# Chainscore/dot-ring

Measured on AMD Instinct MI355X. Metric: ringvrf_proofs_per_sec, higher is better.
Workload: dtype u32

## Files before the change

dot_ring_amd/csrc/capi_msm.hip:

```cpp
#include "capi_internal.hpp"
#include "kernels_g1.hip.h"
#include "kernels_te_msm.hip.h"

using namespace dri;

static MsmKnobs msm_knobs() {
    static const int force_groups = std::getenv("DOTRING_MSM_GROUPS") ? std::atoi(std::getenv("DOTRING_MSM_GROUPS")) : 0;
    static const bool naf_tiling = !(std::getenv("DOTRING_SRS_TILING") && std::strcmp(std::getenv("DOTRING_SRS_TILING"), "rows") == 0);
    return MsmKnobs{g_force_c, force_groups, naf_tiling};
}

namespace {
int msm_reserve(dr_ctx* ctx, const MsmPlan& p) {
    const auto& b = p.bytes;
    for (const auto& r : {std::make_pair(&ctx->counts, b.counts), {&ctx->offsets, b.offsets}, {&ctx->tiles, b.tiles}, {&ctx->perm, b.perm},
                          {&ctx->cells, b.cells}, {&ctx->cell_off, b.cell_off}, {&ctx->buckets, b.buckets}, {&ctx->partial, b.partial},
                          {&ctx->winsum, b.winsum}, {&ctx->heavy, b.heavy}, {&ctx->sorted, b.sorted}, {&ctx->digits, b.digits},
                          {&ctx->cursor, b.cursor}, {&ctx->part_base, b.part_base}, {&ctx->result, b.result}})
        TRY(r.first->reserve(r.second));
    return DR_OK;
}

void exclusive_scan(dr_ctx* ctx, const uint32_t* in, uint32_t* out, size_t count) {
    hipStream_t st = ctx->stream;
    const unsigned nt = div_up(count, dr::SCAN_TILE);
    hipLaunchKernelGGL(dr::k_scan_tiles, dim3(nt), dim3(dr::SCAN_BLOCK), 0, st, in, out, ctx->tiles.as<uint32_t>(), count);
    hipLaunchKernelGGL(dr::k_scan_tile_sums, dim3(1), dim3(dr::SCAN_BLOCK), 0, st, ctx->tiles.as<uint32_t>(), nt, ctx->tiles.as<uint32_t>() + nt);
    hipLaunchKernelGGL(dr::k_scan_add, dim3(div_up(count, 256)), dim3(256), 0, st, out, ctx->tiles.as<uint32_t>(), count);
}

int msm_sort(dr_ctx* ctx, const MsmPlan& p, const uint32_t* d_scalars, const MsmTable* tbl, bool exact, const uint32_t*& part_flag) {
    hipStream_t st = ctx->stream;
    if (p.sort == MsmSort::sets || p.sort == MsmSort::sets_staged) {
        dr::SortSetParams sp{};
        sp.n = (uint32_t)p.n; sp.batch = (uint32_t)p.batch; sp.H = p.H; sp.groups = p.groups; sp.single = p.single ? 1 : 0;
        sp.tbl_stride = p.single ? tbl->stride : 0; sp.tbl_offset = p.single ? tbl->offset : 0; sp.capacity = (uint32_t)p.per_set_digits;
        sp.short_from = p.single ? tbl->short_from : 0xffffffffu; sp.n_short = p.single ? std::min<uint32_t>(tbl->n_short, (uint32_t)p.n) : 0;
        sp.sets = (uint32_t)p.bsets; sp.fold = p.single && tbl->fold_sign ? 1 : 0; sp.n_pad = p.n_pad; sp.digits_per_set = p.digits_per_set;
        return launch(ctx, "k_g1_sort_sets", [&] {
            const auto staged = p.H <= dr::SORT2_SMALL_H ? dr::k_g1_sort_sets_staged<dr::SORT2_SMALL_H, dr::SORT2_CAP_SMALL_H>
                                                         : dr::k_g1_sort_sets_staged<dr::SORT_MAX_H, dr::SORT2_CAP_LARGE_H>;
            if (p.sort == MsmSort::sets_staged)
                hipLaunchKernelGGL(staged, dim3((unsigned)p.bsets), dim3(dr::SORT2_BLOCK), 0, st, d_scalars, p.wt, sp, ctx->digits.as<uint16_t>(),
                                   ctx->counts.as<uint32_t>(), ctx->offsets.as<uint32_t>(), ctx->sorted.as<uint32_t>());
            else
                hipLaunchKernelGGL(dr::k_g1_sort_sets, dim3((unsigned)p.bsets), dim3(dr::SORT_BLOCK), 0, st, d_scalars, p.wt, sp,
                                   ctx->counts.as<uint32_t>(), ctx->offsets.as<uint32_t>(), ctx->sorted.as<uint32_t>());
        });
    }
    if (p.sort == MsmSort::partition) {
        dr::PartParams pp{};
        pp.n = (uint32_t)p.n; pp.H = p.H; pp.groups = p.groups; pp.P = p.part_p; pp.pshift = p.part_shift; pp.tile = p.part_tile;
        pp.tiles_per_set = p.part_tiles_per_set; pp.cap_part = p.part_cap; pp.capacity = (uint32_t)p.per_set_digits;
        pp.tbl_stride = tbl->stride; pp.tbl_offset = tbl->offset;
        for (int w = 0; w < p.wt.W; w++) pp.row[w] = p.wt.row[w];
        const size_t nparts = p.nparts();
        uint32_t* d_flag = ctx->cursor.as<uint32_t>() + nparts;
        const uint32_t* d_exact = nullptr;
        bool fits = true;
        if (exact) {
            std::vector<uint32_t> fill(nparts), at(nparts);
            HIP_TRY(hipMemcpyAsync(fill.data(), ctx->cursor.p, nparts * 4, hipMemcpyDeviceToHost, st));
            HIP_TRY(hipStreamSynchronize(st));
            uint64_t run = 0, most = 0;
            for (size_t q = 0; q < nparts; q++) { at[q] = (uint32_t)run; run += fill[q]; most = std::max<uint64_t>(most, fill[q]); }
            fits = most <= dr::PART_MAX_CHUNKS * (dr::PART_STAGE - dr::PART_SLACK) && run <= nparts * (uint64_t)pp.cap_part;
            if (fits) {
                HIP_TRY(hipMemcpyAsync(ctx->part_base.p, at.data(), nparts * 4, hipMemcpyHostToDevice, st));
                HIP_TRY(hipStreamSynchronize(st));
                d_exact = ctx->part_base.as<uint32_t>();
            }
        }
        if (fits) {
            HIP_TRY(hipMemsetAsync(ctx->cursor.p, 0, (nparts + 1) * 4, st));
            TRY(launch(ctx, "k_g1_part_scatter", [&] {
                hipLaunchKernelGGL(dr::k_g1_part_scatter, dim3((unsigned)(p.bsets * pp.tiles_per_set)), dim3(dr::PART_BLOCK), 0, st, d_scalars, p.wt, pp,
                                   ctx->cursor.as<uint32_t>(), d_exact, ctx->digits.as<uint2>());
            }));
            if (!exact) part_flag = d_flag;
            return launch(ctx, "k_g1_part_sort", [&] {
                hipLaunchKernelGGL(dr::k_g1_part_sort, dim3((unsigned)nparts), dim3(dr::PART_BLOCK), 0, st, ctx->digits.as<uint2>(),
                                   ctx->cursor.as<uint32_t>(), d_exact, pp, d_flag, ctx->counts.as<uint32_t>(), ctx->offsets.as<uint32_t>(),
                                   ctx->sorted.as<uint32_t>());
            });
        }
    }
    HIP_TRY(hipMemsetAsync(ctx->counts.p, 0, p.nbuckets * 4, st));
    HIP_TRY(hipMemsetAsync(ctx->cursor.p, 0, p.nbuckets * 4, st));
    TRY(launch(ctx, "k_g1_digits", [&] {
        hipLaunchKernelGGL(dr::k_g1_digits, dim3(div_up(p.n * p.batch, 256)), dim3(256), 0, st, d_scalars, (uint32_t)p.n,
                           (uint32_t)p.batch, p.wt, p.single ? 1 : 0, p.groups, ctx->digits.as<int32_t>(), ctx->counts.as<uint32_t>());
    }));
    TRY(launch(ctx, "k_scan", [&] { exclusive_scan(ctx, ctx->counts.as<uint32_t>(), ctx->offsets.as<uint32_t>(), p.nbuckets); }));
    return launch(ctx, "k_g1_scatter", [&] {
        hipLaunchKernelGGL(dr::k_g1_scatter, dim3(div_up(p.ndigits, 256)), dim3(256), 0, st, ctx->digits.as<int32_t>(),
                           (uint32_t)p.n, p.windows, p.H, p.single ? p.wt.W : 0, p.wt, p.single ? tbl->stride : 0u, p.single ? tbl->offset : 0u,
// ... 891 lines not shown
```

dot_ring_amd/csrc/kernels_g1.hip.h:

```cpp
#pragma once
#include "dev_types.hpp"
#include "g1.hip.h"
#include "msm_plan.hpp"
#include "msm_recode.hip.h"

namespace dr {

__global__ __launch_bounds__(256) void k_g1_bases_to_mont(uint32_t* bases, uint32_t n) {
    uint32_t i = blockIdx.x * blockDim.x + threadIdx.x;
    if (i >= n) return;
    uint32_t* p = bases + (size_t)i * 24;
    uint32_t wx[12], wy[12];
    load_words12(p, wx);
    load_words12(p + 12, wy);
    store_fq28(p, to_mont28(wx));
    store_fq28(p + 12, to_mont28(wy));
}

__global__ __launch_bounds__(256) void k_g1_synth_bases(uint32_t* bases, uint32_t n, uint32_t first, const uint32_t* seed) {
    uint32_t i = blockIdx.x * blockDim.x + threadIdx.x;
    if (i >= n) return;
    G1Affine s = load_affine(seed, 0);
    uint32_t k = first + i;
    G1Xyzz acc = g1_inf();
// ... 313 lines not shown
    uint32_t i = (uint32_t)(gid % n);
    uint32_t mag = d < 0 ? (uint32_t)(-d) : (uint32_t)d;
    size_t bset = win;
    uint32_t entry = i;
    if (W > 0) {
        bset = (win / W) * groups + (size_t)(((uint64_t)i * groups) / n);
        entry = (uint32_t)wt.row[win % W] * tbl_stride + tbl_offset + i;
    }
    size_t bucket = bset * H + (mag - 1);
    uint32_t pos = offsets[bucket] + atomicAdd(&cursor[bucket], 1u);
    sorted[pos] = entry | (d < 0 ? 0x80000000u : 0u);
}

__global__ __launch_bounds__(256) void k_g1_window_table(const uint32_t* __restrict__ bases, uint32_t n, WindowTable wt, uint32_t pt_words, uint32_t* __restrict__ table) {
    uint32_t i = blockIdx.x * blockDim.x + threadIdx.x;
    if (i >= n) return;
    G1Affine a = load_affine(bases, i);
    G1Xyzz cur = g1_from_affine(a);
#pragma unroll 1
    for (int w = 0; w < wt.W; w++) {
        if (w > 0) {
#pragma unroll 1
            for (int j = 0; j < wt.width[w - 1]; j++) cur = g1_dbl(cur);
            a = g1_to_affine_dev(cur);
        }
        store_affine(table + ((size_t)w * n + i) * (pt_words - 24), (size_t)w * n + i, a);
    }
}

__global__ __launch_bounds__(128) void k_g1_bit_table(const uint32_t* __restrict__ bases, uint32_t n, uint32_t rows, uint32_t pt_words, uint32_t* __restrict__ table) {
    uint32_t i = blockIdx.x * blockDim.x + threadIdx.x;
    if (i >= n) return;
    G1Affine a = load_affine(bases, i);
#pragma unroll 1
    for (uint32_t s = 0; s < rows; s++) {
        if (s > 0 && !a.inf) a = g1_to_affine_dev(g1_dbl_affine(a));
        store_affine(table + ((size_t)s * n + i) * (pt_words - 24), (size_t)s * n + i, a);
    }
}

DR_DEV uint32_t digit_bin(const WindowTable& wt, int w, uint32_t mag, uint32_t& row) {
    row = wt.row[w];
    return mag - 1u;
}

constexpr int SORT_BLOCK = 256;

struct SortSetParams {
    uint32_t n, batch, H, groups;
    int single;
    uint32_t tbl_stride, tbl_offset;
    uint32_t capacity;
    uint32_t short_from, n_short;
    uint32_t n_pad, digits_per_set;
    uint32_t sets;
    int fold;
};

DR_DEV void load_scalar_mod_r(const uint32_t* __restrict__ scalars, size_t idx, uint32_t (&k)[9]) {
    const uint4* q = reinterpret_cast<const uint4*>(scalars + idx * 8);
    uint4 lo = q[0], hi = q[1];
    k[0] = lo.x; k[1] = lo.y; k[2] = lo.z; k[3] = lo.w; k[4] = hi.x; k[5] = hi.y; k[6] = hi.z; k[7] = hi.w;
    k[8] = 0;
    constexpr uint32_t R[8] = {0x00000001u, 0xffffffffu, 0xfffe5bfeu, 0x53bda402u, 0x09a1d805u, 0x3339d808u, 0x299d7d48u, 0x73eda753u};
#pragma unroll 1
    for (int it = 0; it < 2; it++) {
        uint32_t d[8], borrow = 0;
#pragma unroll
        for (int j = 0; j < 8; j++) d[j] = subb(k[j], R[j], borrow);
#pragma unroll
        for (int j = 0; j < 8; j++) k[j] = borrow ? k[j] : d[j];
    }
}

DR_DEV bool scalar_fold_sign(uint32_t (&k)[9]) {
    constexpr uint32_t R[8] = {0x00000001u, 0xffffffffu, 0xfffe5bfeu, 0x53bda402u, 0x09a1d805u, 0x3339d808u, 0x299d7d48u, 0x73eda753u};
    constexpr uint32_t HALF[8] = {0x80000000u, 0x7fffffffu, 0x7fff2dffu, 0xa9ded201u, 0x04d0ec02u, 0x199cec04u, 0x94cebea4u, 0x39f6d3a9u};
    uint32_t borrow = 0, d[8];
#pragma unroll
    for (int j = 0; j < 8; j++) (void)subb(HALF[j], k[j], borrow);
    const bool neg = borrow != 0;
    borrow = 0;
#pragma unroll
    for (int j = 0; j < 8; j++) d[j] = subb(R[j], k[j], borrow);
#pragma unroll
    for (int j = 0; j < 8; j++) k[j] = neg ? d[j] : k[j];
    return neg;
}


__global__ __launch_bounds__(SORT_BLOCK) void k_g1_sort_sets(const uint32_t* __restrict__ scalars, WindowTable wt, SortSetParams sp,
                                                             uint32_t* __restrict__ counts, uint32_t* __restrict__ offsets,
                                                             uint32_t* __restrict__ sorted) {
    __shared__ uint32_t bins[SORT_MAX_H];
    __shared__ uint32_t smem[SORT_BLOCK / 64];
    const uint32_t H = sp.H, HB = sp.H, set = blockIdx.x;
    uint32_t b, i_lo, i_hi;
    int w_lo, w_hi;
    if (sp.single) {
        b = set / sp.groups;
        uint32_t g = set % sp.groups;
        const uint32_t n_eff = b >= sp.short_from ? sp.n_short : sp.n;
        i_lo = (uint32_t)(((uint64_t)g * n_eff + sp.groups - 1) / sp.groups);
        i_hi = (uint32_t)(((uint64_t)(g + 1) * n_eff + sp.groups - 1) / sp.groups);
        w_lo = 0; w_hi = wt.W;
    } else {
        const uint32_t sw = set / sp.groups, g = set % sp.groups;
        b = sw / wt.W;
// ... 7 lines not shown
        uint32_t k[9];
        load_scalar_mod_r(scalars, (size_t)b * sp.n + i, k);
        if (sp.fold) (void)scalar_fold_sign(k);
        if (wt.odd == 2) {
            for_each_wnaf_digit(k, wt, [&](int, uint32_t, int32_t d) { atomicAdd(&bins[((uint32_t)(d < 0 ? -d : d) - 1u) >> 1], 1u); });
            continue;
        }
        for_each_digit(k, wt, w_lo, w_hi, [&](int w, int32_t d) {
            uint32_t row;
            atomicAdd(&bins[digit_bin(wt, w, (uint32_t)(d < 0 ? -d : d), row)], 1u);
        });
    }
    __syncthreads();
    const uint32_t per = (HB + SORT_BLOCK - 1) / SORT_BLOCK, lo = threadIdx.x * per < HB ? threadIdx.x * per : HB, hi = lo + per < HB ? lo + per : HB;
    uint32_t local = 0;
    for (uint32_t j = lo; j < hi; j++) {
        uint32_t c = bins[j];
        counts[(size_t)set * H + j] = c;
        local += c;
    }
    uint32_t total;
    uint32_t run = block_exclusive_scan(local, smem, total);
    const uint32_t base = set * sp.capacity;
    for (uint32_t j = lo; j < hi; j++) {
        uint32_t c = bins[j];
        bins[j] = run;
        offsets[(size_t)set * H + j] = base + run;
        run += c;
    }
    __syncthreads();
    for (uint32_t i = i_lo + threadIdx.x; i < i_hi; i += SORT_BLOCK) {
        uint32_t k[9];
        load_scalar_mod_r(scalars, (size_t)b * sp.n + i, k);
        const bool neg = sp.fold ? scalar_fold_sign(k) : false;
        if (wt.odd == 2) {
            for_each_wnaf_digit(k, wt, [&](int j, uint32_t o, int32_t d) {
                const uint32_t pos = atomicAdd(&bins[((uint32_t)(d < 0 ? -d : d) - 1u) >> 1], 1u);
                const uint32_t entry = ((uint32_t)wt.row[j] + o) * sp.tbl_stride + sp.tbl_offset + i;
                sorted[base + pos] = entry | ((d < 0) != neg ? 0x80000000u : 0u);
            });
            continue;
        }
        for_each_digit(k, wt, w_lo, w_hi, [&](int w, int32_t d) {
            uint32_t row;
            uint32_t pos = atomicAdd(&bins[digit_bin(wt, w, (uint32_t)(d < 0 ? -d : d), row)], 1u);
            uint32_t entry = sp.single ? row * sp.tbl_stride + sp.tbl_offset + i : i;
            sorted[base + pos] = entry | ((d < 0) != neg ? 0x80000000u : 0u);
        });
    }
}

template <uint32_t MAX_H, uint32_t SORT2_CAP>
__global__ __launch_bounds__(SORT2_BLOCK) void k_g1_sort_sets_staged(const uint32_t* __restrict__ scalars, WindowTable wt, SortSetParams sp,
                                                                    uint16_t* __restrict__ digits16, uint32_t* __restrict__ counts,
                                                                    uint32_t* __restrict__ offsets, uint32_t* __restrict__ sorted) {
    constexpr uint32_t SORT2_CHUNK = SORT2_CAP - SORT2_SLACK;
    __shared__ uint32_t bins[MAX_H];
    __shared__ uint32_t stage[SORT2_CAP];
    __shared__ uint32_t cs[SORT2_MAX_CHUNKS + 1], jb[SORT2_MAX_CHUNKS + 1];
    __shared__ uint32_t smem[SORT2_BLOCK / 64];
    const uint32_t H = sp.H, set = blockIdx.x, tid = threadIdx.x;
    uint32_t b, i_lo, i_hi;
    int w_lo, w_hi;
    if (sp.single) {
        b = set / sp.groups;
        uint32_t g = set % sp.groups;
        const uint32_t n_eff = b >= sp.short_from ? sp.n_short : sp.n;
        i_lo = (uint32_t)(((uint64_t)g * n_eff + sp.groups - 1) / sp.groups);
        i_hi = (uint32_t)(((uint64_t)(g + 1) * n_eff + sp.groups - 1) / sp.groups);
        w_lo = 0; w_hi = wt.W;
    } else {
        const uint32_t sw = set / sp.groups, g = set % sp.groups;
        b = sw / wt.W;
        w_lo = (int)(sw % wt.W); w_hi = w_lo + 1;
        i_lo = (uint32_t)(((uint64_t)g * sp.n + sp.groups - 1) / sp.groups);
        i_hi = (uint32_t)(((uint64_t)(g + 1) * sp.n + sp.groups - 1) / sp.groups);
    }
    const uint32_t n_set = i_hi - i_lo, n_pad = (n_set + 7u) & ~7u, rows = (uint32_t)(w_hi - w_lo);
    uint16_t* dg = digits16 + (size_t)set * sp.digits_per_set;
    for (uint32_t j = tid; j < H; j += SORT2_BLOCK) bins[j] = 0;
    for (uint32_t k = tid; k <= SORT2_MAX_CHUNKS; k += SORT2_BLOCK) { cs[k] = 0xffffffffu; jb[k] = H; }
    __syncthreads();
    for (uint32_t ii = tid; ii < n_pad; ii += SORT2_BLOCK) {
        if (ii < n_set) {
            uint32_t k[9];
            load_scalar_mod_r(scalars, (size_t)b * sp.n + i_lo + ii, k);
            const bool neg = sp.fold ? scalar_fold_sign(k) : false;
            if (wt.odd == 2) {
                for_each_wnaf_digit<true>(k, wt, [&](int j, uint32_t o, int32_t d) {
                    uint32_t enc = WNAF_EMPTY16;
                    if (d != 0) {
                        const uint32_t bin = ((uint32_t)(d < 0 ? -d : d) - 1u) >> 1;
                        atomicAdd(&bins[bin], 1u);
                        enc = bin | (o << 11) | ((d < 0) != neg ? 0x8000u : 0u);
                    }
                    dg[(size_t)j * n_pad + ii] = (uint16_t)enc;
                });
            } else
            for_each_digit<true>(k, wt, w_lo, w_hi, [&](int w, int32_t d) {
                const uint32_t mag = (uint32_t)(d < 0 ? -d : d);
                uint32_t row, enc = mag;
                if (d != 0) {
                    atomicAdd(&bins[digit_bin(wt, w, mag, row)], 1u);
                }
                dg[(size_t)(w - w_lo) * n_pad + ii] = (uint16_t)(enc | ((d < 0) != neg && d != 0 ? 0x8000u : 0u));
            });
        } else {
            for (uint32_t r = 0; r < rows; r++) dg[(size_t)r * n_pad + ii] = wt.odd == 2 ? (uint16_t)WNAF_EMPTY16 : (uint16_t)0;
        }
    }
    __syncthreads();
    const uint32_t per = (H + SORT2_BLOCK - 1) / SORT2_BLOCK, lo = tid * per < H ? tid * per : H, hi = lo + per < H ? lo + per : H;
    uint32_t local = 0;
    for (uint32_t j = lo; j < hi; j++) {
        uint32_t c = bins[j];
        counts[(size_t)set * H + j] = c;
        local += c;
    }
    uint32_t total;
    uint32_t run = block_exclusive_scan<SORT2_BLOCK>(local, smem, total);
    const uint32_t base = set * sp.capacity;
    const uint32_t K = (total + SORT2_CHUNK - 1) / SORT2_CHUNK;
    for (uint32_t j = lo; j < hi; j++) {
        uint32_t c = bins[j];
        bins[j] = run;
        offsets[(size_t)set * H + j] = base + run;
        const uint32_t k = run / SORT2_CHUNK;
        atomicMin(&jb[k], j);
        atomicMin(&cs[k], run);
        run += c;
    }
    __syncthreads();
    if (tid == 0) {
        cs[K] = total; jb[K] = H;
        for (int k = (int)K - 1; k >= 0; k--) {
            if (cs[k] == 0xffffffffu) cs[k] = cs[k + 1];
            if (jb[k] > jb[k + 1]) jb[k] = jb[k + 1];
        }
    }
    __syncthreads();
    const uint32_t tbl = sp.single ? sp.tbl_offset : 0u;
    for (uint32_t k = 0; k < K; k++) {
        const uint32_t j_lo = jb[k], j_hi = jb[k + 1], p_lo = cs[k], p_hi = cs[k + 1], c0 = k * SORT2_CHUNK;
        if (j_lo < j_hi) {
            const uint32_t nv = n_pad / 8, nvec = rows * nv;
            const uint4* vecs = reinterpret_cast<const uint4*>(dg);
            uint32_t r = 0, v = tid;
            for (uint32_t idx = tid; idx < nvec; idx += SORT2_BLOCK, v += SORT2_BLOCK) {
                while (v >= nv) { v -= nv; r++; }
                const uint32_t row_entry = (sp.single ? (uint32_t)wt.row[w_lo + (int)r] * sp.tbl_stride : 0u) + tbl + i_lo;
                {
                    const uint4 q = vecs[idx];
                    const uint32_t words[4] = {q.x, q.y, q.z, q.w};
#pragma unroll
                    for (int t = 0; t < 8; t++) {
                        const uint32_t dd = (words[t >> 1] >> (16 * (t & 1))) & 0xffffu;
                        const uint32_t j = wt.odd == 2 ? (((dd >> 11) & 15u) == 15u ? 0xffffffffu : (dd & 0x7ffu)) : (dd & 0x7fffu) - 1u;
                        if (j >= j_lo && j < j_hi) {
                            uint32_t up = 0;
                            if (wt.odd == 2) {
                                up = ((dd >> 11) & 15u) * sp.tbl_stride;
                            }
                            const uint32_t pos = atomicAdd(&bins[j], 1u);
                            const uint32_t entry = (row_entry + up + v * 8 + (uint32_t)t) | ((dd & 0x8000u) << 16);
                            const uint32_t rel = pos - c0;
                            if (rel < SORT2_CAP) stage[rel] = entry;
                            else sorted[base + pos] = entry;
                        }
                    }
                }
            }
        }
        __syncthreads();
        const uint32_t r_lo = p_lo - c0, r_hi = (p_hi - c0) < SORT2_CAP ? (p_hi - c0) : SORT2_CAP;
        for (uint32_t rel = r_lo + tid; rel < r_hi; rel += SORT2_BLOCK) sorted[base + c0 + rel] = stage[rel];
        __syncthreads();
    }
}

struct PartParams {
    uint32_t n, H, groups, tiles_per_set, P, pshift;
    uint32_t tile;
    uint32_t cap_part;
    uint32_t capacity;
    uint32_t tbl_stride, tbl_offset;
    uint8_t row[32];
};

DR_DEV void part_set_range(const PartParams& pp, uint32_t set, uint32_t& b, uint32_t& i_lo, uint32_t& i_hi) {
    b = set / pp.groups;
    const uint32_t g = set % pp.groups;
    i_lo = (uint32_t)(((uint64_t)g * pp.n + pp.groups - 1) / pp.groups);
    i_hi = (uint32_t)(((uint64_t)(g + 1) * pp.n + pp.groups - 1) / pp.groups);
}

DR_DEV uint32_t lds_count_aggregated(uint32_t* bins, uint32_t j) {
    const uint32_t lane = threadIdx.x & 63u;
    unsigned long long todo = __ballot(1);
    uint32_t pos = 0;
    bool done = false;
#pragma unroll 1
    for (int round = 0; round < 4 && todo; round++) {
        const int leader = __builtin_ctzll(todo);
        const uint32_t j0 = (uint32_t)__shfl((int)j, leader, 64);
        const unsigned long long same = __ballot(!done && j == j0);
        if (__popcll(same) < 2 && round == 0) break;
        uint32_t base = 0;
        if ((int)lane == leader) base = atomicAdd(&bins[j0], (uint32_t)__popcll(same));
        base = (uint32_t)__shfl((int)base, leader, 64);
        if (!done && j == j0) { pos = base + (uint32_t)__popcll(same & ((1ull << lane) - 1ull)); done = true; }
        todo &= ~same;
    }
    if (!done) pos = atomicAdd(&bins[j], 1u);
    return pos;
}

__global__ __launch_bounds__(PART_BLOCK) void k_g1_part_scatter(const uint32_t* __restrict__ scalars, WindowTable wt, PartParams pp,
                                                                uint32_t* __restrict__ part_fill, const uint32_t* __restrict__ exact_base,
                                                                uint2* __restrict__ streams) {
    constexpr int WAVES = PART_BLOCK / 64;
    __shared__ uint32_t stage[PART_TILE_ENTRIES];
    __shared__ uint32_t cnt[PART_MAX_P];
    __shared__ uint32_t pbase[PART_MAX_P + 1], gbase[PART_MAX_P];
    __shared__ uint32_t smem[PART_BLOCK / 64];
    const uint32_t set = blockIdx.x / pp.tiles_per_set, tile = blockIdx.x % pp.tiles_per_set, tid = threadIdx.x, wave = tid >> 6;
    const bool per_wave = pp.P * WAVES <= PART_MAX_P;
    uint32_t b, i_lo, i_hi;
    part_set_range(pp, set, b, i_lo, i_hi);
// ... 622 lines not shown
```

dot_ring_amd/csrc/msm_plan.hpp:

```cpp
#pragma once
#include <algorithm>
#include <cmath>
#include <cstddef>
#include <cstdint>

#include "dev_types.hpp"

namespace dr {

constexpr int SCAN_BLOCK = 256, SCAN_ITEMS = 8, SCAN_TILE = SCAN_BLOCK * SCAN_ITEMS;
constexpr uint32_t SORT_MAX_H = 8192;
constexpr int SORT2_BLOCK = 1024;
constexpr uint32_t SORT2_SLACK = 2048, SORT2_MAX_CHUNKS = 64;
constexpr uint32_t SORT2_CAP_SMALL_H = 36864, SORT2_CAP_LARGE_H = 28672, SORT2_SMALL_H = 2048;
constexpr int PART_BLOCK = 1024;
constexpr uint32_t PART_TILE_ENTRIES = 32768, PART_MAX_P = 1024, PART_MAX_HP = 1024, PART_STAGE = 36864, PART_SLACK = 2048, PART_MAX_CHUNKS = 64;
constexpr int SZ_BLOCK = 256, SZ_ITEMS = 8, SZ_TILE = SZ_BLOCK * SZ_ITEMS, SZ_CLASSES = 256;
constexpr uint32_t G1_HEAVY_SLOTS = 2048;
constexpr int RS_BLOCK = 64, RS_GROUP = 4;
constexpr int WS_BLOCK = 256;

constexpr int MIN_WINDOW = 7, MAX_WINDOW = 16, MAX_TABLE_WINDOW = 22;
inline bool forced_window_ok(int c) { return c >= MIN_WINDOW && c <= MAX_WINDOW; }
inline bool table_window_ok(int c) { return c >= MIN_WINDOW && c <= MAX_TABLE_WINDOW; }

inline int pick_window(size_t n) {
    int best = MIN_WINDOW;
    double best_cost = 1e300;
    for (int c = MIN_WINDOW; c <= MAX_WINDOW; c++) {
        int W = (256 + c - 1) / c;
        double cost = (double)W * ((double)n + 2.8 * (double)(1u << (c - 1)) + 40.0 * (double)((1u << (c - 1)) / 16 + 1));
        if (cost < best_cost) { best_cost = cost; best = c; }
    }
    return best;
}

inline int pick_window_latency(size_t n) {
    int best = 7;
    double best_t = 1e300;
    for (int c = 7; c <= 13; c++) {
        const int W = (256 + c - 1) / c;
        const double H = (double)(1u << (c - 1));
        if ((double)W * H > 131072.0) continue;
        const double m = (double)n / H;
        const double reduce = H >= 256.0 ? 15.0 * (2.0 * std::min(8.0, std::max(1.0, H / 1024.0)) + 17.0)
                                         : 15.0 * (8.0 + 1.5 * (c - 3)) + 15.0 * (std::log2(std::max(H / 4.0, 2.0)) + 4.0);
        const double t = 11.0 * (m + 3.0 * std::sqrt(m) + 1.0) + reduce;
        if (t < best_t) { best_t = t; best = c; }
    }
    return best;
}

inline WindowTable make_window_table(int c, int bits = 256) {
    WindowTable wt;
    wt.W = (bits + c - 1) / c;
    int base = bits / wt.W, rem = bits % wt.W;
    wt.cmax = base + (rem ? 1 : 0);
    int bit = 0;
    for (int w = 0; w < wt.W; w++) {
        int width = base + (w >= wt.W - rem ? 1 : 0);
        wt.start[w] = (uint8_t)bit, wt.width[w] = (uint8_t)width, wt.row[w] = (uint8_t)w;
        bit += width;
    }
    wt.odd = 0;
    return wt;
}

// ... 1 lines not shown

struct MsmTable {
    const uint32_t* table = nullptr;
    dr::WindowTable wt{};
    uint32_t pt_words = 24;
    bool bit_rows = false;
    int naf_delta = -2;
    uint32_t stride = 0, offset = 0;
    uint32_t short_from = 0xffffffffu, n_short = 0;
    bool fold_sign = false;
};

struct MsmKnobs { int force_c = 0, force_groups = 0; bool naf_tiling = true; };

constexpr size_t L4_BELOW = (size_t)1 << 15;

struct Tiling { bool naf; int c, slots; double digits; };

inline Tiling tiling_for(const MsmTable& t, size_t n, size_t batch, bool naf_tiling) {
    Tiling none{false, 0, 0, 0.0};
    if (!t.table || !t.bit_rows || t.naf_delta == -1 || batch < 256 || n == 0 || !naf_tiling) return none;
    const int cn = t.wt.cmax;
    const int lo = t.naf_delta >= 0 ? cn + t.naf_delta : cn - 1, hi = t.naf_delta >= 0 ? cn + t.naf_delta : cn + 2;
    Tiling best = none;
    double best_cost = 0;
    for (int w = lo; w <= hi; w++) {
        if (w < 9 || w > 13) continue;
        const size_t H = (size_t)1 << (w - 2), slots = (256 + w - 1) / w;
        if (batch * (H / 16) < L4_BELOW) continue;
        if ((n + 64) * slots > ((size_t)1 << 20) || batch * (n + 64) * slots >= (1ull << 32)) continue;
        const double digits = 256.0 / (w + 1) + 0.55;
        if (t.naf_delta < 0 && (double)n * digits / (double)H > 160.0) continue;
        const double cost = (double)n * digits + 1.5 * (double)H;
        if (!best.naf || cost < best_cost) { best = Tiling{true, w, (int)slots, digits}; best_cost = cost; }
    }
    return best;
}

enum class MsmSort { sets, sets_staged, partition, global };
enum class MsmReduce { set_scan, levels, wg_scan, chunks, chunks_two_stage };
enum class MsmFinish { group_sum, device_copy, host_horner, device_horner };

struct MsmPlan {
    const char* error = nullptr;
    size_t n = 0, batch = 0;
    bool single = false;
    dr::WindowTable wt{};
    uint32_t H = 0, L = 0, T = 0, groups = 1;
    size_t windows = 0, bsets = 0, nbuckets = 0, ndigits = 0, per_set_scalars = 0, per_set_digits = 0;
    MsmSort sort = MsmSort::global;
    MsmReduce reduce = MsmReduce::chunks;
    MsmFinish finish = MsmFinish::group_sum;
    uint32_t n_pad = 0, digits_per_set = 0;
    uint32_t part_p = 1, part_shift = 0;
    uint32_t part_tile = 0, part_tiles_per_set = 0, part_cap = 0;
    uint32_t ws_per_lane = 1, ws_span = 0;
    size_t wg_per_set = 0, wg_count = 0;
    size_t szblocks = 0, ncells = 0;
    struct { size_t counts, offsets, tiles, perm, cells, cell_off, buckets, partial, winsum, heavy, sorted, digits, cursor, part_base, result; }
        bytes{};
    size_t nparts() const { return bsets * (size_t)part_p; }
};

inline MsmPlan msm_shape(size_t n, size_t batch, const MsmTable* tbl, const MsmKnobs& k, bool allow_naf) {
    MsmPlan p;
    p.n = n, p.batch = batch, p.single = tbl != nullptr && tbl->table != nullptr;
    if (p.single) {
        const Tiling tl = allow_naf ? tiling_for(*tbl, n, batch, k.naf_tiling) : Tiling{false, 0, 0, 0.0};
        if (tl.naf) {
            const int shift = tl.slots * tl.c - 256;
            p.wt.W = tl.slots, p.wt.cmax = tl.c, p.wt.odd = 2;
            for (int j = 0; j < p.wt.W; j++)
                p.wt.start[j] = (uint8_t)(tl.c * j), p.wt.row[j] = (uint8_t)(j ? tl.c * j - shift : 0), p.wt.width[j] = (uint8_t)tl.c;
        } else {
            p.wt = tbl->wt;
        }
        p.H = 1u << (p.wt.cmax - (tl.naf ? 2 : 1));
    } else {
        const bool latency_bound = batch == 1 && n <= 32768;
        p.wt = dr::make_window_table(dr::forced_window_ok(k.force_c) ? k.force_c : latency_bound ? dr::pick_window_latency(n) : dr::pick_window(n));
        p.H = 1u << (p.wt.cmax - 1);
    }
    p.L = std::min<uint32_t>(p.H, 16u);
    if (p.single) {
        const size_t target_lanes = n >= ((size_t)1 << 19) ? 524288 : 262144;
        while (p.groups < 64 && batch * p.groups * (size_t)p.H < target_lanes && n / (p.groups * 2) >= 64) p.groups *= 2;
        if (k.force_groups > 0 && batch == 1 && n / (size_t)k.force_groups >= 64) p.groups = (uint32_t)k.force_groups;
    }
    p.windows = batch * (size_t)p.wt.W;
    p.bsets = p.single ? batch * p.groups : p.windows;
    if (p.single && p.L == 16 && p.H >= 256 && p.H <= 4096 && p.bsets * (size_t)(p.H / 16) < L4_BELOW) p.L = 4;
    if (!p.single && p.L == 16 && p.H >= 16 && p.bsets * (size_t)(p.H / 16) < ((size_t)1 << 12)) p.L = 4;
    p.T = p.H / p.L;
    p.per_set_scalars = p.single ? (n + p.groups - 1) / p.groups : n;
    p.per_set_digits = p.single ? p.per_set_scalars * (size_t)p.wt.W : n;
    const bool lds_sort = p.H <= dr::SORT_MAX_H && p.bsets >= 64 && p.per_set_digits <= (1u << 20) && p.bsets * p.per_set_digits < (1ull << 32);
    p.sort = lds_sort ? MsmSort::sets : MsmSort::global;
    const bool setscan = p.L == 16 && p.T >= 8 && p.T <= 256 && p.bsets >= 256;
    p.reduce = setscan ? MsmReduce::set_scan : MsmReduce::chunks;
    return p;
}

inline MsmPlan plan_msm(size_t n, size_t batch, const MsmTable* tbl, const MsmKnobs& k) {
    MsmPlan p = msm_shape(n, batch, tbl, k, true);
    if (p.wt.odd && !(p.sort == MsmSort::sets && p.reduce == MsmReduce::set_scan)) p = msm_shape(n, batch, tbl, k, false);
    const uint32_t H = p.H, T = p.T, W = (uint32_t)p.wt.W;
    const size_t bsets = p.bsets;
    if (p.single && ((uint64_t)p.wt.row[W - 1] + p.wt.cmax + 1) * tbl->stride >= (1ull << 31)) { p.error = "window table too large"; return p; }
    p.nbuckets = bsets * (size_t)H, p.ndigits = p.windows * n;
    if (p.nbuckets >= (1ull << 32) || p.ndigits >= (1ull << 32)) { p.error = "MSM batch too large for one launch (split the batch)"; return p; }

    if (p.sort == MsmSort::sets) {
        const uint32_t stage_chunk = (H <= dr::SORT2_SMALL_H ? dr::SORT2_CAP_SMALL_H : dr::SORT2_CAP_LARGE_H) - dr::SORT2_SLACK;
        if (p.per_set_digits >= 4096 && p.per_set_digits / stage_chunk + 1 <= dr::SORT2_MAX_CHUNKS) {
            p.sort = MsmSort::sets_staged;
            p.n_pad = (uint32_t)((p.per_set_scalars + 7) & ~(size_t)7), p.digits_per_set = p.n_pad * (p.single ? W : 1u);
        }
    }
    const size_t chunk = dr::PART_STAGE - dr::PART_SLACK;
    while (p.part_p < dr::PART_MAX_P && (H / p.part_p > dr::PART_MAX_HP || p.per_set_digits / p.part_p > chunk - chunk / 16)) p.part_p *= 2;
    while ((H >> p.part_shift) > p.part_p) p.part_shift++;
    if (p.sort == MsmSort::global && p.single && batch == 1 && W <= 32 && H >= p.part_p && H / p.part_p <= dr::PART_MAX_HP &&
        p.per_set_digits / p.part_p <= 48 * chunk && bsets * p.per_set_digits < (1ull << 32) && p.per_set_digits >= 65536) {
        p.sort = MsmSort::partition;
        p.part_tile = std::min<uint32_t>(2048, dr::PART_TILE_ENTRIES / W);
        p.part_tiles_per_set = (uint32_t)((p.per_set_scalars + p.part_tile - 1) / p.part_tile);
        p.part_cap = (uint32_t)std::min<size_t>(p.per_set_digits, std::max<size_t>(4 * p.per_set_digits / p.part_p, 65536));
    }

    const bool setscan = p.reduce == MsmReduce::set_scan;
    const bool leveled = p.L == 16 && H >= 256 && bsets * (size_t)(H / 16) >= ((size_t)1 << 18);
    const bool plain_one = !p.single && batch == 1 && !setscan && !leveled && H >= 256 && !p.wt.odd;
    if (plain_one) p.ws_per_lane = std::min<uint32_t>(8u, std::max<uint32_t>(1u, H / 1024u));
    else while (p.ws_per_lane < 8 && bsets * (size_t)H > (size_t)65536 * p.ws_per_lane) p.ws_per_lane *= 2;
    p.ws_span = dr::WS_BLOCK * p.ws_per_lane;
    const bool few_table = p.single && batch <= 32 && !setscan && !leveled && H >= 256 && !p.wt.odd && bsets * (size_t)H <= ((size_t)1 << 19);
    const bool wgscan = (plain_one || few_table || (!setscan && !leveled && p.single && batch == 1 && H >= 8192)) && H % p.ws_span == 0;
    p.wg_per_set = H / p.ws_span, p.wg_count = bsets * p.wg_per_set;
    if (!setscan) p.reduce = leveled ? MsmReduce::levels : wgscan ? MsmReduce::wg_scan
                           : T > 512 && T % 256 == 0 ? MsmReduce::chunks_two_stage : MsmReduce::chunks;
    if (p.single) p.finish = wgscan || p.groups > 1 || batch == 1 ? MsmFinish::group_sum : MsmFinish::device_copy;
    else p.finish = batch == 1 ? MsmFinish::host_horner : MsmFinish::device_horner;

    p.szblocks = (p.nbuckets + dr::SZ_TILE - 1) / dr::SZ_TILE, p.ncells = (size_t)dr::SZ_CLASSES * p.szblocks;
    auto& b = p.bytes;
    b.counts = b.perm = p.nbuckets * 4, b.offsets = (p.nbuckets + 1) * 4;
    b.tiles = (size_t)((std::max(p.ncells, p.nbuckets) + dr::SCAN_TILE - 1) / dr::SCAN_TILE + 1) * 4;
    b.cells = p.ncells * 4, b.cell_off = (p.ncells + 2) * 4;
    b.buckets = p.nbuckets * 192;
    size_t levels = 0;
    for (uint32_t m = H; m > 16; m /= 16) levels += 2 * bsets * (m / 16);
    b.partial = std::max((bsets * T + bsets * (T / 256 + 1)) * 192, p.reduce == MsmReduce::set_scan ? 2 * bsets * T * 192
                         : p.reduce == MsmReduce::wg_scan ? 2 * p.wg_count * 192 : p.reduce == MsmReduce::levels ? levels * 192 : 0);
    b.winsum = bsets * 192;
    b.heavy = (p.ndigits / 1024 + p.ndigits / 4096 + dr::G1_HEAVY_SLOTS / 2 + 64) * 192;
    const bool global = p.sort == MsmSort::global, part = p.sort == MsmSort::partition;
    b.sorted = global ? p.ndigits * 4 : bsets * p.per_set_digits * 4;
    b.digits = global ? p.ndigits * 4 : part ? p.nparts() * p.part_cap * 8 : bsets * (size_t)p.digits_per_set * 2;
    b.cursor = global ? p.nbuckets * 4 : part ? std::max(p.nparts() + 1, p.nbuckets) * 4 : 0;
    b.part_base = part ? p.nparts() * 4 : 0;
    b.result = batch > 1 ? batch * 192 : 0;
    return p;
}
```

dot_ring_amd/csrc/msm_recode.hip.h:

```cpp
#pragma once
#include <cstdint>

#include "dev_types.hpp"

#if defined(__HIPCC__)
#define DR_RECODE_FN __device__ __forceinline__
#else
#define DR_RECODE_FN static inline
#endif

namespace dr {

template <bool WITH_ZEROS = false, class F>
DR_RECODE_FN void for_each_digit(const uint32_t (&k)[9], const WindowTable& wt, int w_lo, int w_hi, F&& f) {
    uint32_t carry = 0;
    int w = 0;
#pragma unroll
    for (int li = 0; li < 8; li++) {
        const uint64_t two = (uint64_t)k[li] | ((uint64_t)k[li + 1] << 32);
        while (w < w_hi && (wt.start[w] >> 5) == li) {
            const int c = wt.width[w], sh = wt.start[w] & 31;
            const uint32_t half = 1u << (c - 1);
            uint32_t raw = ((uint32_t)(two >> sh) & ((1u << c) - 1)) + carry;
            int32_t d;
            if (raw > half) { d = (int32_t)raw - (int32_t)(1u << c); carry = 1; }
            else { d = (int32_t)raw; carry = 0; }
            if (w >= w_lo && (WITH_ZEROS || d != 0)) f(w, d);
            w++;
        }
    }
}

constexpr uint32_t WNAF_EMPTY16 = 0x7800u;
constexpr uint32_t WNAF_ZONE = 3;
template <bool WITH_ZEROS = false, class F>
DR_RECODE_FN void for_each_wnaf_digit(const uint32_t (&k)[9], const WindowTable& wt, F&& f) {
    const uint32_t w = (uint32_t)wt.cmax, wmask = (1u << w) - 1u, L = (uint32_t)wt.W * w, shift = L - 256u;
    uint32_t K[10];
    K[0] = k[0] << shift;
#pragma unroll
    for (int i = 1; i < 9; i++) K[i] = shift ? (k[i] << shift) | (k[i - 1] >> (32u - shift)) : k[i];
    K[9] = 0;
    uint32_t c = 0, r = 0;
    int j = 0;
#pragma unroll
    for (int li = 0; li < 9; li++) {
        const uint64_t two = (uint64_t)K[li] | ((uint64_t)K[li + 1] << 32);
        while (j < wt.W && (wt.start[j] >> 5) == li) {
            const uint32_t chunk = (uint32_t)(two >> (wt.start[j] & 31));
            const uint32_t m = (((c ? ~chunk : chunk) & wmask) >> r) << r;
            if (m) {
                const uint32_t o = (uint32_t)__builtin_ctz(m);
                const uint32_t R = L - ((uint32_t)wt.start[j] + o);
                uint32_t a = w;
                if (R <= WNAF_ZONE * w) {
                    const uint32_t q = (R + w - 1u) / w;
                    a = (R + q - 1u) / q;
                }
                const uint32_t v = ((chunk >> o) & ((1u << a) - 1u)) + c;
                int32_t d;
                if (v > (1u << (a - 1))) { d = (int32_t)v - (int32_t)(1u << a); c = 1; }
                else { d = (int32_t)v; c = 0; }
                f(j, j == 0 ? o - shift : o, d);
                r = o + a - w;
            } else {
                if (WITH_ZEROS) f(j, 0u, 0);
                r = 0;
            }
            j++;
        }
    }
}

}
```

Before: 17680.

## Replace dense 16-bit digit matrix with bucket-range packed records in staged sort

The staged per-set sort now writes only nonzero digits as packed 32-bit records (sign, bucket low bits, row, index) into per-range regions whose sizes come from a host-side sampled digit profile. The scatter pass reads only each chunk's ranges instead of rescanning the whole dense digit matrix once per chunk. This is meant to cut the redundant global reads and filtering in the old multi-chunk scan. If a region overflows, the kernel recomputes exact offsets and redoes the recode pass, and it falls back to plain sets sort when the bits do not fit.

```diff
diff --git a/dot_ring_amd/csrc/capi_msm.hip b/dot_ring_amd/csrc/capi_msm.hip
--- a/dot_ring_amd/csrc/capi_msm.hip
+++ b/dot_ring_amd/csrc/capi_msm.hip
@@ -36,12 +36,14 @@
         sp.n = (uint32_t)p.n; sp.batch = (uint32_t)p.batch; sp.H = p.H; sp.groups = p.groups; sp.single = p.single ? 1 : 0;
         sp.tbl_stride = p.single ? tbl->stride : 0; sp.tbl_offset = p.single ? tbl->offset : 0; sp.capacity = (uint32_t)p.per_set_digits;
         sp.short_from = p.single ? tbl->short_from : 0xffffffffu; sp.n_short = p.single ? std::min<uint32_t>(tbl->n_short, (uint32_t)p.n) : 0;
-        sp.sets = (uint32_t)p.bsets; sp.fold = p.single && tbl->fold_sign ? 1 : 0; sp.n_pad = p.n_pad; sp.digits_per_set = p.digits_per_set;
+        sp.sets = (uint32_t)p.bsets; sp.fold = p.single && tbl->fold_sign ? 1 : 0;
+        sp.i_bits = p.i_bits; sp.rb_bits = p.rb_bits; sp.nranges = p.nranges; sp.region_words = p.region_words;
+        std::copy(p.region_at, p.region_at + dr::SORT2_MAX_RANGES + 1, sp.region_at);
         return launch(ctx, "k_g1_sort_sets", [&] {
             const auto staged = p.H <= dr::SORT2_SMALL_H ? dr::k_g1_sort_sets_staged<dr::SORT2_SMALL_H, dr::SORT2_CAP_SMALL_H>
                                                          : dr::k_g1_sort_sets_staged<dr::SORT_MAX_H, dr::SORT2_CAP_LARGE_H>;
             if (p.sort == MsmSort::sets_staged)
-                hipLaunchKernelGGL(staged, dim3((unsigned)p.bsets), dim3(dr::SORT2_BLOCK), 0, st, d_scalars, p.wt, sp, ctx->digits.as<uint16_t>(),
+                hipLaunchKernelGGL(staged, dim3((unsigned)p.bsets), dim3(dr::SORT2_BLOCK), 0, st, d_scalars, p.wt, sp, ctx->digits.as<uint32_t>(),
                                    ctx->counts.as<uint32_t>(), ctx->offsets.as<uint32_t>(), ctx->sorted.as<uint32_t>());
             else
                 hipLaunchKernelGGL(dr::k_g1_sort_sets, dim3((unsigned)p.bsets), dim3(dr::SORT_BLOCK), 0, st, d_scalars, p.wt, sp,
diff --git a/dot_ring_amd/csrc/kernels_g1.hip.h b/dot_ring_amd/csrc/kernels_g1.hip.h
--- a/dot_ring_amd/csrc/kernels_g1.hip.h
+++ b/dot_ring_amd/csrc/kernels_g1.hip.h
@@ -389,8 +389,9 @@
     uint32_t tbl_stride, tbl_offset;
     uint32_t capacity;
     uint32_t short_from, n_short;
-    uint32_t n_pad, digits_per_set;
     uint32_t sets;
+    uint32_t i_bits, rb_bits, nranges, region_words;
+    uint32_t region_at[SORT2_MAX_RANGES + 1];
     int fold;
 };
 
@@ -504,13 +505,13 @@
 
 template <uint32_t MAX_H, uint32_t SORT2_CAP>
 __global__ __launch_bounds__(SORT2_BLOCK) void k_g1_sort_sets_staged(const uint32_t* __restrict__ scalars, WindowTable wt, SortSetParams sp,
-                                                                    uint16_t* __restrict__ digits16, uint32_t* __restrict__ counts,
+                                                                    uint32_t* __restrict__ records, uint32_t* __restrict__ counts,
                                                                     uint32_t* __restrict__ offsets, uint32_t* __restrict__ sorted) {
-    constexpr uint32_t SORT2_CHUNK = SORT2_CAP - SORT2_SLACK;
     __shared__ uint32_t bins[MAX_H];
     __shared__ uint32_t stage[SORT2_CAP];
-    __shared__ uint32_t cs[SORT2_MAX_CHUNKS + 1], jb[SORT2_MAX_CHUNKS + 1];
+    __shared__ uint32_t fill[SORT2_MAX_RANGES], rat[SORT2_MAX_RANGES + 1], rpos[SORT2_MAX_RANGES + 1], ck[SORT2_MAX_RANGES + 1];
     __shared__ uint32_t smem[SORT2_BLOCK / 64];
+    __shared__ uint32_t over, nck;
     const uint32_t H = sp.H, set = blockIdx.x, tid = threadIdx.x;
     uint32_t b, i_lo, i_hi;
     int w_lo, w_hi;
@@ -528,40 +529,49 @@
         i_lo = (uint32_t)(((uint64_t)g * sp.n + sp.groups - 1) / sp.groups);
         i_hi = (uint32_t)(((uint64_t)(g + 1) * sp.n + sp.groups - 1) / sp.groups);
     }
-    const uint32_t n_set = i_hi - i_lo, n_pad = (n_set + 7u) & ~7u, rows = (uint32_t)(w_hi - w_lo);
-    uint16_t* dg = digits16 + (size_t)set * sp.digits_per_set;
+    const uint32_t n_set = i_hi - i_lo, R = sp.nranges, rbb = sp.rb_bits, ib = sp.i_bits, rowb = sort_row_bits(sp.single != 0);
+    const uint32_t rbmask = (1u << rbb) - 1u;
+    uint32_t* rec = records + (size_t)set * sp.region_words;
     for (uint32_t j = tid; j < H; j += SORT2_BLOCK) bins[j] = 0;
-    for (uint32_t k = tid; k <= SORT2_MAX_CHUNKS; k += SORT2_BLOCK) { cs[k] = 0xffffffffu; jb[k] = H; }
-    __syncthreads();
-    for (uint32_t ii = tid; ii < n_pad; ii += SORT2_BLOCK) {
-        if (ii < n_set) {
+    for (uint32_t r = tid; r <= R; r += SORT2_BLOCK) { rat[r] = sp.region_at[r]; if (r < R) fill[r] = 0; }
+    __syncthreads();
+#pragma unroll 1
+    for (int exact = 0; exact < 2; exact++) {
+        for (uint32_t ii = tid; ii < n_set; ii += SORT2_BLOCK) {
             uint32_t k[9];
             load_scalar_mod_r(scalars, (size_t)b * sp.n + i_lo + ii, k);
             const bool neg = sp.fold ? scalar_fold_sign(k) : false;
-            if (wt.odd == 2) {
-                for_each_wnaf_digit<true>(k, wt, [&](int j, uint32_t o, int32_t d) {
-                    uint32_t enc = WNAF_EMPTY16;
-                    if (d != 0) {
-                        const uint32_t bin = ((uint32_t)(d < 0 ? -d : d) - 1u) >> 1;
-                        atomicAdd(&bins[bin], 1u);
-                        enc = bin | (o << 11) | ((d < 0) != neg ? 0x8000u : 0u);
-                    }
-                    dg[(size_t)j * n_pad + ii] = (uint16_t)enc;
+            auto put = [&](uint32_t bin, uint32_t row, bool minus) {
+                if (!exact) atomicAdd(&bins[bin], 1u);
+                const uint32_t r = bin >> rbb;
+                const uint32_t at = rat[r] + atomicAdd(&fill[r], 1u);
+                if (at < rat[r + 1]) rec[at] = sort_pack(minus ? 1u : 0u, bin & rbmask, row, ii, rowb, ib);
+            };
+            if (wt.odd == 2)
+                for_each_wnaf_digit(k, wt, [&](int j, uint32_t o, int32_t d) {
+                    put(((uint32_t)(d < 0 ? -d : d) - 1u) >> 1, (uint32_t)wt.row[j] + o, (d < 0) != neg);
                 });
-            } else
-            for_each_digit<true>(k, wt, w_lo, w_hi, [&](int w, int32_t d) {
-                const uint32_t mag = (uint32_t)(d < 0 ? -d : d);
-                uint32_t row, enc = mag;
-                if (d != 0) {
-                    atomicAdd(&bins[digit_bin(wt, w, mag, row)], 1u);
-                }
-                dg[(size_t)(w - w_lo) * n_pad + ii] = (uint16_t)(enc | ((d < 0) != neg && d != 0 ? 0x8000u : 0u));
-            });
-        } else {
-            for (uint32_t r = 0; r < rows; r++) dg[(size_t)r * n_pad + ii] = wt.odd == 2 ? (uint16_t)WNAF_EMPTY16 : (uint16_t)0;
-        }
-    }
-    __syncthreads();
+            else
+                for_each_digit(k, wt, w_lo, w_hi, [&](int w, int32_t d) {
+                    put((uint32_t)(d < 0 ? -d : d) - 1u, sp.single ? (uint32_t)wt.row[w] : 0u, (d < 0) != neg);
+                });
+        }
+        __syncthreads();
+        if (tid == 0) {
+            uint32_t o = 0;
+            for (uint32_t r = 0; r < R; r++) o |= fill[r] > rat[r + 1] - rat[r] ? 1u : 0u;
+            if (o) {
+                uint32_t at = 0;
+                for (uint32_t r = 0; r < R; r++) { rat[r] = at; at += fill[r]; }
+                rat[R] = at;
+            }
+            over = o;
+        }
+        __syncthreads();
+        if (!over) break;
+        for (uint32_t r = tid; r < R; r += SORT2_BLOCK) fill[r] = 0;
+        __syncthreads();
+    }
     const uint32_t per = (H + SORT2_BLOCK - 1) / SORT2_BLOCK, lo = tid * per < H ? tid * per : H, hi = lo + per < H ? lo + per : H;
     uint32_t local = 0;
     for (uint32_t j = lo; j < hi; j++) {
@@ -572,60 +582,56 @@
     uint32_t total;
     uint32_t run = block_exclusive_scan<SORT2_BLOCK>(local, smem, total);
     const uint32_t base = set * sp.capacity;
-    const uint32_t K = (total + SORT2_CHUNK - 1) / SORT2_CHUNK;
     for (uint32_t j = lo; j < hi; j++) {
         uint32_t c = bins[j];
         bins[j] = run;
         offsets[(size_t)set * H + j] = base + run;
-        const uint32_t k = run / SORT2_CHUNK;
-        atomicMin(&jb[k], j);
-        atomicMin(&cs[k], run);
         run += c;
     }
-    __syncthreads();
     if (tid == 0) {
-        cs[K] = total; jb[K] = H;
-        for (int k = (int)K - 1; k >= 0; k--) {
-            if (cs[k] == 0xffffffffu) cs[k] = cs[k + 1];
-            if (jb[k] > jb[k + 1]) jb[k] = jb[k + 1];
-        }
-    }
-    __syncthreads();
-    const uint32_t tbl = sp.single ? sp.tbl_offset : 0u;
-    for (uint32_t k = 0; k < K; k++) {
-        const uint32_t j_lo = jb[k], j_hi = jb[k + 1], p_lo = cs[k], p_hi = cs[k + 1], c0 = k * SORT2_CHUNK;
-        if (j_lo < j_hi) {
-            const uint32_t nv = n_pad / 8, nvec = rows * nv;
-            const uint4* vecs = reinterpret_cast<const uint4*>(dg);
-            uint32_t r = 0, v = tid;
-            for (uint32_t idx = tid; idx < nvec; idx += SORT2_BLOCK, v += SORT2_BLOCK) {
-                while (v >= nv) { v -= nv; r++; }
-                const uint32_t row_entry = (sp.single ? (uint32_t)wt.row[w_lo + (int)r] * sp.tbl_stride : 0u) + tbl + i_lo;
-                {
-                    const uint4 q = vecs[idx];
-                    const uint32_t words[4] = {q.x, q.y, q.z, q.w};
-#pragma unroll
-                    for (int t = 0; t < 8; t++) {
-                        const uint32_t dd = (words[t >> 1] >> (16 * (t & 1))) & 0xffffu;
-                        const uint32_t j = wt.odd == 2 ? (((dd >> 11) & 15u) == 15u ? 0xffffffffu : (dd & 0x7ffu)) : (dd & 0x7fffu) - 1u;
-                        if (j >= j_lo && j < j_hi) {
-                            uint32_t up = 0;
-                            if (wt.odd == 2) {
-                                up = ((dd >> 11) & 15u) * sp.tbl_stride;
-                            }
-                            const uint32_t pos = atomicAdd(&bins[j], 1u);
-                            const uint32_t entry = (row_entry + up + v * 8 + (uint32_t)t) | ((dd & 0x8000u) << 16);
-                            const uint32_t rel = pos - c0;
-                            if (rel < SORT2_CAP) stage[rel] = entry;
-                            else sorted[base + pos] = entry;
-                        }
-                    }
+        uint32_t at = 0, c = 0;
+        for (uint32_t r = 0; r < R; r++) { rpos[r] = at; at += fill[r]; }
+        rpos[R] = at;
+        for (uint32_t r = 0; r < R;) {
+            ck[c++] = r;
+            uint32_t n = fill[r++];
+            while (r < R && n + fill[r] <= SORT2_CAP) n += fill[r++];
+        }
+        ck[c] = R;
+        nck = c;
+    }
+    __syncthreads();
+    const uint32_t entry0 = (sp.single ? sp.tbl_offset : 0u) + i_lo, stride = sp.single ? sp.tbl_stride : 0u;
+    for (uint32_t c = 0; c < nck; c++) {
+        const uint32_t c0 = rpos[ck[c]], cn = rpos[ck[c + 1]] - c0;
+        uint32_t r = ck[c];
+        for (uint32_t q0 = tid; q0 < cn; q0 += 4 * SORT2_BLOCK) {
+            uint32_t v[4], rr[4];
+#pragma unroll
+            for (int u = 0; u < 4; u++) {
+                const uint32_t q = c0 + q0 + (uint32_t)u * SORT2_BLOCK;
+                rr[u] = 0xffffffffu;
+                if (q < c0 + cn) {
+                    while (q >= rpos[r + 1]) r++;
+                    rr[u] = r;
+                    v[u] = rec[rat[r] + (q - rpos[r])];
                 }
             }
+#pragma unroll
+            for (int u = 0; u < 4; u++) {
+                if (rr[u] == 0xffffffffu) continue;
+                uint32_t neg, jr, row, ii;
+                sort_unpack(v[u], rowb, ib, rbb, neg, jr, row, ii);
+                const uint32_t pos = atomicAdd(&bins[(rr[u] << rbb) + jr], 1u);
+                const uint32_t entry = (row * stride + entry0 + ii) | (neg << 31);
+                const uint32_t rel = pos - c0;
+                if (rel < SORT2_CAP) stage[rel] = entry;
+                else sorted[base + pos] = entry;
+            }
         }
         __syncthreads();
-        const uint32_t r_lo = p_lo - c0, r_hi = (p_hi - c0) < SORT2_CAP ? (p_hi - c0) : SORT2_CAP;
-        for (uint32_t rel = r_lo + tid; rel < r_hi; rel += SORT2_BLOCK) sorted[base + c0 + rel] = stage[rel];
+        const uint32_t r_hi = cn < SORT2_CAP ? cn : SORT2_CAP;
+        for (uint32_t rel = tid; rel < r_hi; rel += SORT2_BLOCK) sorted[base + c0 + rel] = stage[rel];
         __syncthreads();
     }
 }
diff --git a/dot_ring_amd/csrc/msm_plan.hpp b/dot_ring_amd/csrc/msm_plan.hpp
--- a/dot_ring_amd/csrc/msm_plan.hpp
+++ b/dot_ring_amd/csrc/msm_plan.hpp
@@ -3,8 +3,12 @@
 #include <cmath>
 #include <cstddef>
 #include <cstdint>
+#include <cstring>
+#include <mutex>
+#include <vector>
 
 #include "dev_types.hpp"
+#include "msm_recode.hip.h"
 
 namespace dr {
 
@@ -13,6 +17,7 @@
 constexpr int SORT2_BLOCK = 1024;
 constexpr uint32_t SORT2_SLACK = 2048, SORT2_MAX_CHUNKS = 64;
 constexpr uint32_t SORT2_CAP_SMALL_H = 36864, SORT2_CAP_LARGE_H = 28672, SORT2_SMALL_H = 2048;
+constexpr uint32_t SORT2_MAX_RANGES = 64, SORT2_RANGE_BITS = 8;
 constexpr int PART_BLOCK = 1024;
 constexpr uint32_t PART_TILE_ENTRIES = 32768, PART_MAX_P = 1024, PART_MAX_HP = 1024, PART_STAGE = 36864, PART_SLACK = 2048, PART_MAX_CHUNKS = 64;
 constexpr int SZ_BLOCK = 256, SZ_ITEMS = 8, SZ_TILE = SZ_BLOCK * SZ_ITEMS, SZ_CLASSES = 256;
@@ -120,6 +125,9 @@
     MsmReduce reduce = MsmReduce::chunks;
     MsmFinish finish = MsmFinish::group_sum;
     uint32_t n_pad = 0, digits_per_set = 0;
+    uint32_t i_bits = 0, rb_bits = 0, nranges = 0;
+    uint32_t region_words = 0;
+    uint32_t region_at[dr::SORT2_MAX_RANGES + 1] = {};
     uint32_t part_p = 1, part_shift = 0;
     uint32_t part_tile = 0, part_tiles_per_set = 0, part_cap = 0;
     uint32_t ws_per_lane = 1, ws_span = 0;
@@ -169,6 +177,62 @@
     return p;
 }
 
+DR_RECODE_FN uint32_t sort_row_bits(bool single) { return single ? 8u : 0u; }
+DR_RECODE_FN uint32_t sort_pack(uint32_t neg, uint32_t jr, uint32_t row, uint32_t ii, uint32_t row_bits, uint32_t i_bits) {
+    return (neg << 31) | (jr << (row_bits + i_bits)) | (row << i_bits) | ii;
+}
+DR_RECODE_FN void sort_unpack(uint32_t rec, uint32_t row_bits, uint32_t i_bits, uint32_t rb_bits, uint32_t& neg, uint32_t& jr, uint32_t& row, uint32_t& ii) {
+    neg = rec >> 31, jr = (rec >> (row_bits + i_bits)) & ((1u << rb_bits) - 1u), row = (rec >> i_bits) & ((1u << row_bits) - 1u), ii = rec & ((1u << i_bits) - 1u);
+}
+
+inline std::vector<double> range_profile(const dr::WindowTable& wt, bool single, uint32_t H, uint32_t rb_bits) {
+    struct Entry { dr::WindowTable wt; bool single; uint32_t H, rb_bits; std::vector<double> prof; };
+    static std::mutex mu;
+    static std::vector<Entry> cache;
+    std::lock_guard<std::mutex> lock(mu);
+    for (const Entry& e : cache)
+        if (e.single == single && e.H == H && e.rb_bits == rb_bits && std::memcmp(&e.wt, &wt, sizeof wt) == 0) return e.prof;
+    const uint32_t R = H >> rb_bits, M = 2048, WW = single ? 1u : (uint32_t)wt.W;
+    std::vector<double> prof(R, 0.0);
+    uint64_t x = 0x9e3779b97f4a7c15ull;
+    for (int half = 0; half < 2; half++) {
+        std::vector<uint32_t> cnt((size_t)WW * R, 0);
+        for (uint32_t s = 0; s < M; s++) {
+            uint32_t k[9];
+            for (int i = 0; i < 8; i++) { x ^= x << 13; x ^= x >> 7; x ^= x << 17; k[i] = (uint32_t)(x >> 16); }
+            k[7] %= half ? 0x39f6d3a9u : 0x73eda753u;
+            k[8] = 0;
+            if (wt.odd == 2)
+                dr::for_each_wnaf_digit(k, wt, [&](int, uint32_t, int32_t d) { cnt[((((uint32_t)(d < 0 ? -d : d) - 1u) >> 1) >> rb_bits)]++; });
+            else
+                dr::for_each_digit(k, wt, 0, wt.W, [&](int w, int32_t d) { cnt[(single ? 0u : (uint32_t)w) * R + (((uint32_t)(d < 0 ? -d : d) - 1u) >> rb_bits)]++; });
+        }
+        for (uint32_t w = 0; w < WW; w++)
+            for (uint32_t r = 0; r < R; r++) prof[r] = std::max(prof[r], (double)cnt[(size_t)w * R + r] / M);
+    }
+    cache.push_back(Entry{wt, single, H, rb_bits, prof});
+    return prof;
+}
+
+inline void sort_regions(MsmPlan& p) {
+    uint32_t i_bits = 1;
+    while ((1ull << i_bits) < p.per_set_scalars) i_bits++;
+    const uint32_t row_bits = sort_row_bits(p.single), log2h = (uint32_t)__builtin_ctz(p.H);
+    if (row_bits + i_bits + 5 > 31) return;
+    const uint32_t rb_bits = std::min({dr::SORT2_RANGE_BITS, 31u - row_bits - i_bits, log2h});
+    const uint32_t R = p.H >> rb_bits;
+    if (R > dr::SORT2_MAX_RANGES) return;
+    const std::vector<double> prof = range_profile(p.wt, p.single, p.H, rb_bits);
+    uint64_t at = 0;
+    for (uint32_t r = 0; r < R; r++) {
+        p.region_at[r] = (uint32_t)at;
+        at += ((uint64_t)std::ceil(1.1 * prof[r] * (double)p.per_set_scalars) + 256 + 3) & ~3ull;
+    }
+    p.region_at[R] = (uint32_t)at;
+    p.region_words = (uint32_t)((std::max<uint64_t>(at, p.per_set_digits) + 3) & ~3ull);
+    p.i_bits = i_bits, p.rb_bits = rb_bits, p.nranges = R;
+}
+
 inline MsmPlan plan_msm(size_t n, size_t batch, const MsmTable* tbl, const MsmKnobs& k) {
     MsmPlan p = msm_shape(n, batch, tbl, k, true);
     if (p.wt.odd && !(p.sort == MsmSort::sets && p.reduce == MsmReduce::set_scan)) p = msm_shape(n, batch, tbl, k, false);
@@ -183,6 +247,8 @@
         if (p.per_set_digits >= 4096 && p.per_set_digits / stage_chunk + 1 <= dr::SORT2_MAX_CHUNKS) {
             p.sort = MsmSort::sets_staged;
             p.n_pad = (uint32_t)((p.per_set_scalars + 7) & ~(size_t)7), p.digits_per_set = p.n_pad * (p.single ? W : 1u);
+            sort_regions(p);
+            if (!p.nranges) p.sort = MsmSort::sets;
         }
     }
     const size_t chunk = dr::PART_STAGE - dr::PART_SLACK;
@@ -224,7 +290,7 @@
     b.heavy = (p.ndigits / 1024 + p.ndigits / 4096 + dr::G1_HEAVY_SLOTS / 2 + 64) * 192;
     const bool global = p.sort == MsmSort::global, part = p.sort == MsmSort::partition;
     b.sorted = global ? p.ndigits * 4 : bsets * p.per_set_digits * 4;
-    b.digits = global ? p.ndigits * 4 : part ? p.nparts() * p.part_cap * 8 : bsets * (size_t)p.digits_per_set * 2;
+    b.digits = global ? p.ndigits * 4 : part ? p.nparts() * p.part_cap * 8 : p.sort == MsmSort::sets_staged ? bsets * (size_t)p.region_words * 4 : 0;
     b.cursor = global ? p.nbuckets * 4 : part ? std::max(p.nparts() + 1, p.nbuckets) * 4 : 0;
     b.part_base = part ? p.nparts() * 4 : 0;
     b.result = batch > 1 ? batch * 192 : 0;
diff --git a/dot_ring_amd/csrc/msm_recode.hip.h b/dot_ring_amd/csrc/msm_recode.hip.h
--- a/dot_ring_amd/csrc/msm_recode.hip.h
+++ b/dot_ring_amd/csrc/msm_recode.hip.h
@@ -4,7 +4,7 @@
 #include "dev_types.hpp"
 
 #if defined(__HIPCC__)
-#define DR_RECODE_FN __device__ __forceinline__
+#define DR_RECODE_FN __host__ __device__ __forceinline__
 #else
 #define DR_RECODE_FN static inline
 #endif
@@ -31,7 +31,6 @@
     }
 }
 
-constexpr uint32_t WNAF_EMPTY16 = 0x7800u;
 constexpr uint32_t WNAF_ZONE = 3;
 template <bool WITH_ZEROS = false, class F>
 DR_RECODE_FN void for_each_wnaf_digit(const uint32_t (&k)[9], const WindowTable& wt, F&& f) {
```

Measured after the change: 17600, median of 6. About the same (-0.4%).
